# cloneofsimo/paint-with-words-sd

Measured on NVIDIA H100. Metric: unet_steps_per_sec_512sq_cfg, higher is better.
Workload: dtype f16

## Files before the change

paint_with_words_sd_b200/csrc/attn_tc.cuh:

```cuda
#pragma once
#include "mma_sm90.cuh"
#include "pww_common.cuh"
#include "xattn_core.cuh"

namespace pww {
namespace fa {

constexpr int kThreads = core::kThreads;
constexpr int kBM = core::kBM;
constexpr int kBN = 64;

template <int D>
struct Cfg {
  using T_ = core::Tile<D>;
  static constexpr uint32_t KVBYTES = kBN * T_::LD * 2;
  static constexpr uint32_t OFF_KV = T_::QBYTES;
  static constexpr uint32_t SMEM = T_::QBYTES + 2 * 2 * KVBYTES;
  static_assert(SMEM <= 232448, "shared memory budget");
};

template <typename E>
struct Params {
  const E* q;
  const E* k;
  const E* v;
  E* out;
  int B, H, N;
  int64_t bs, rs;
  int64_t o_bs, o_rs;
  float scale;
};

template <int D, typename E>
constexpr int kMinBlocks = (D == 80 && std::is_same_v<E, __nv_bfloat16>) ? 1 : 0;

template <int D, typename E>
__global__ void __launch_bounds__(kThreads, kMinBlocks<D, E>) attn_fwd_kernel(const Params<E> p) {
  using C = core::Tile<D>;
  using CF = Cfg<D>;
  extern __shared__ __align__(128) unsigned char smem[];
  const uint32_t smem0 = ptx::smem_u32(smem);
  const int warp = threadIdx.x >> 5, lane = threadIdx.x & 31;
  const int qtiles = (p.N + kBM - 1) / kBM;
  const int bh = blockIdx.x / qtiles, qt = blockIdx.x - bh * qtiles;
  const int b = bh / p.H, h = bh - b * p.H;
  const int row_base = qt * kBM;
  const E* qb = p.q + (int64_t)b * p.bs + h * D;
  const E* kb = p.k + (int64_t)b * p.bs + h * D;
  const E* vb = p.v + (int64_t)b * p.bs + h * D;
  const int ntiles = (p.N + kBN - 1) / kBN;
  auto issue_kv = [&](int j) {
    const uint32_t st = smem0 + CF::OFF_KV + (j & 1) * 2 * CF::KVBYTES;
    const int rows = p.N - j * kBN < kBN ? p.N - j * kBN : kBN;
    core::load_rows<D>(st, kb + (int64_t)j * kBN * p.rs, p.rs, kBN, rows);
    core::load_rows<D>(st + CF::KVBYTES, vb + (int64_t)j * kBN * p.rs, p.rs, kBN, rows);
    ptx::cp_async_commit();
  };
  {
    const int rows = p.N - row_base < kBM ? p.N - row_base : kBM;
    core::load_rows<D>(smem0, qb + (int64_t)row_base * p.rs, p.rs, kBM, rows);
  }
  issue_kv(0);
  uint32_t qa[C::KS][4];
  float o[C::NT][4], m0, m1, l0, l1;
  core::warp_online_begin<D>(o, m0, m1, l0, l1);
  const float sl2 = p.scale * 1.4426950408889634f;
  const uint32_t qs = smem0 + (uint32_t)(warp * 16 * C::LD) * 2u;
#pragma unroll 1
  for (int jt = 0; jt < ntiles; ++jt) {
    if (jt + 1 < ntiles) {
      issue_kv(jt + 1);
      ptx::cp_async_wait<1>();
    } else {
      ptx::cp_async_wait<0>();
    }
    __syncthreads();
    if (jt == 0) {
#pragma unroll
      for (int kk = 0; kk < C::KS; ++kk)
        ptx::ldsm_x4(qs + (uint32_t)((lane & 15) * C::LD + kk * 16 + (lane >> 4) * 8) * 2u, qa[kk][0], qa[kk][1], qa[kk][2], qa[kk][3]);
    }
    const uint32_t ks = smem0 + CF::OFF_KV + (jt & 1) * 2 * CF::KVBYTES, vs = ks + CF::KVBYTES;
    float s[kBN / 8][4];
#pragma unroll
    for (int j = 0; j < kBN / 8; ++j) s[j][0] = s[j][1] = s[j][2] = s[j][3] = 0.f;
#pragma unroll
    for (int kk = 0; kk < C::KS; ++kk) {
#pragma unroll
      for (int jp = 0; jp < kBN / 16; ++jp) {
        const int t = 16 * jp + (lane & 7) + ((lane >> 4) << 3), d = kk * 16 + ((lane >> 3) & 1) * 8;
        uint32_t b0, b1, b2, b3;
        ptx::ldsm_x4(ks + (uint32_t)(t * C::LD + d) * 2u, b0, b1, b2, b3);
        ptx::mma16816<E>(s[2 * jp], qa[kk], b0, b1);
        ptx::mma16816<E>(s[2 * jp + 1], qa[kk], b2, b3);
      }
    }
    core::warp_online_chunk<D, E>(s, p.N - jt * kBN, sl2, vs, lane, o, m0, m1, l0, l1);
    __syncthreads();
  }
  core::warp_online_end<D>(o, l0, l1);
  core::warp_store<D>(o, smem + warp * 16 * C::LD * 2, lane, p.out + (int64_t)b * p.o_bs + h * D, p.o_rs,
                      row_base + warp * 16, p.N);
}

template <int D, typename E>
cudaError_t launch(const void* q, const void* k, const void* v, void* out, int B, int H, int N, int64_t bs, int64_t rs,
                   int64_t o_bs, int64_t o_rs, float scale, cudaStream_t s) {
  using CF = Cfg<D>;
  Params<E> p;
  p.q = (const E*)q; p.k = (const E*)k; p.v = (const E*)v; p.out = (E*)out;
  p.B = B; p.H = H; p.N = N; p.bs = bs; p.rs = rs; p.o_bs = o_bs; p.o_rs = o_rs; p.scale = scale;
  const cudaError_t e = allow_dynamic_smem<attn_fwd_kernel<D, E>>(CF::SMEM);
  if (e != cudaSuccess) return e;
  const long long grid = (long long)B * H * ((N + kBM - 1) / kBM);
  if (grid > 0x7fffffffLL) return cudaErrorInvalidConfiguration;
  attn_fwd_kernel<D, E><<<(unsigned)grid, kThreads, CF::SMEM, s>>>(p);
  return cudaGetLastError();
}

}
}
```

paint_with_words_sd_b200/csrc/mma_sm90.cuh:

```cuda
#pragma once
#include <cuda_runtime.h>
#include <stdint.h>

#include <type_traits>

#include "pww_common.cuh"

namespace pww {
namespace ptx {

__device__ __forceinline__ uint32_t smem_u32(const void* p) { return (uint32_t)__cvta_generic_to_shared(p); }

__device__ __forceinline__ void cp_async16(uint32_t dst, const void* src, uint32_t src_bytes) {
  asm volatile("cp.async.cg.shared.global [%0], [%1], 16, %2;" ::"r"(dst), "l"(src), "r"(src_bytes) : "memory");
}
__device__ __forceinline__ void cp_async_commit() { asm volatile("cp.async.commit_group;" ::: "memory"); }
template <int N>
__device__ __forceinline__ void cp_async_wait() { asm volatile("cp.async.wait_group %0;" ::"n"(N) : "memory"); }

__device__ __forceinline__ void ldsm_x4(uint32_t addr, uint32_t& r0, uint32_t& r1, uint32_t& r2, uint32_t& r3) {
  asm volatile("ldmatrix.sync.aligned.m8n8.x4.shared.b16 {%0, %1, %2, %3}, [%4];"
               : "=r"(r0), "=r"(r1), "=r"(r2), "=r"(r3) : "r"(addr));
}
__device__ __forceinline__ void ldsm_x4_t(uint32_t addr, uint32_t& r0, uint32_t& r1, uint32_t& r2, uint32_t& r3) {
  asm volatile("ldmatrix.sync.aligned.m8n8.x4.trans.shared.b16 {%0, %1, %2, %3}, [%4];"
               : "=r"(r0), "=r"(r1), "=r"(r2), "=r"(r3) : "r"(addr));
}
__device__ __forceinline__ void ldsm_x2_t(uint32_t addr, uint32_t& r0, uint32_t& r1) {
  asm volatile("ldmatrix.sync.aligned.m8n8.x2.trans.shared.b16 {%0, %1}, [%2];" : "=r"(r0), "=r"(r1) : "r"(addr));
}

template <typename E>
__device__ __forceinline__ void mma16816(float* c, const uint32_t* a, uint32_t b0, uint32_t b1) {
  static_assert(std::is_same_v<E, __half> || std::is_same_v<E, __nv_bfloat16>, "fp16 or bf16 operands");
  if constexpr (std::is_same_v<E, __half>) {
    asm volatile(
        "mma.sync.aligned.m16n8k16.row.col.f32.f16.f16.f32 {%0, %1, %2, %3}, {%4, %5, %6, %7}, {%8, %9}, "
        "{%0, %1, %2, %3};"
        : "+f"(c[0]), "+f"(c[1]), "+f"(c[2]), "+f"(c[3])
        : "r"(a[0]), "r"(a[1]), "r"(a[2]), "r"(a[3]), "r"(b0), "r"(b1));
  } else {
    asm volatile(
        "mma.sync.aligned.m16n8k16.row.col.f32.bf16.bf16.f32 {%0, %1, %2, %3}, {%4, %5, %6, %7}, {%8, %9}, "
        "{%0, %1, %2, %3};"
        : "+f"(c[0]), "+f"(c[1]), "+f"(c[2]), "+f"(c[3])
        : "r"(a[0]), "r"(a[1]), "r"(a[2]), "r"(a[3]), "r"(b0), "r"(b1));
  }
}

__device__ __forceinline__ float ex2(float x) {
  float y;
  asm("ex2.approx.ftz.f32 %0, %1;" : "=f"(y) : "f"(x));
  return y;
}
template <typename E>
__device__ __forceinline__ uint32_t pack2(float lo, float hi) {
  const typename Elem<E>::E2 h = Elem<E>::from_float2(lo, hi);
  return *reinterpret_cast<const uint32_t*>(&h);
}
template <typename E>
__device__ __forceinline__ float2 unpack2(uint32_t v) {
  return Elem<E>::to_float2(*reinterpret_cast<const typename Elem<E>::E2*>(&v));
}
__device__ __forceinline__ unsigned long long ld_acquire_gpu_u64(const unsigned long long* p) {
  unsigned long long v;
  asm volatile("ld.acquire.gpu.global.u64 %0, [%1];" : "=l"(v) : "l"(p) : "memory");
  return v;
}

}
}
```

paint_with_words_sd_b200/csrc/xattn_core.cuh:

```cuda
#pragma once
#include "mma_sm90.cuh"
#include "pww_common.cuh"

namespace pww {
namespace core {

constexpr int kBM = 128;
constexpr int kTP = 80;
constexpr int kWarps = 8;
constexpr int kThreads = kWarps * 32;

template <int D>
struct Tile {
  static_assert(D == 40 || D == 64 || D == 80 || D == 160, "head dims of SD1.5 (40 / 80 / 160) and SD2.x (64)");
  static constexpr int DP = (D + 15) / 16 * 16;
  static constexpr int LD = DP + 8;
  static constexpr int KS = DP / 16;
  static constexpr int NT = D / 8;
  static constexpr uint32_t QBYTES = kBM * LD * 2;
  static constexpr uint32_t KBYTES = kTP * LD * 2;
};

template <int D, typename E>
__device__ __forceinline__ void load_rows(uint32_t dst, const E* src, int64_t rs, int nrows, int valid) {
  using C = Tile<D>;
  constexpr int CH = C::DP / 8, DCH = D / 8;
  for (int idx = threadIdx.x; idx < nrows * CH; idx += blockDim.x) {
    const int r = idx / CH, c = idx - r * CH;
    const bool ok = r < valid && c < DCH;
    ptx::cp_async16(dst + (uint32_t)(r * C::LD + c * 8) * 2u, ok ? (const void*)(src + (int64_t)r * rs + c * 8) : (const void*)src,
                    ok ? 16u : 0u);
  }
}

template <int D, typename E>
__device__ __forceinline__ void warp_qk(uint32_t qs, uint32_t ks, int lane, float (&s)[10][4]) {
  using C = Tile<D>;
#pragma unroll
  for (int j = 0; j < 10; ++j) s[j][0] = s[j][1] = s[j][2] = s[j][3] = 0.f;
#pragma unroll
  for (int kk = 0; kk < C::KS; ++kk) {
    uint32_t a[4];
    ptx::ldsm_x4(qs + (uint32_t)((lane & 15) * C::LD + kk * 16 + (lane >> 4) * 8) * 2u, a[0], a[1], a[2], a[3]);
#pragma unroll
    for (int jp = 0; jp < 5; ++jp) {
      const int t = 16 * jp + (lane & 7) + ((lane >> 4) << 3), d = kk * 16 + ((lane >> 3) & 1) * 8;
      uint32_t b0, b1, b2, b3;
      ptx::ldsm_x4(ks + (uint32_t)(t * C::LD + d) * 2u, b0, b1, b2, b3);
      ptx::mma16816<E>(s[2 * jp], a, b0, b1);
      ptx::mma16816<E>(s[2 * jp + 1], a, b2, b3);
    }
  }
}

__device__ __forceinline__ int tok(int j, int e, int lane) { return 8 * j + 2 * (lane & 3) + (e & 1); }

template <int D, typename E>
__device__ __forceinline__ void warp_store(const float (&o)[Tile<D>::NT][4], unsigned char* stage, int lane, E* out,
                                           int64_t o_rs, int row0, int N) {
  using C = Tile<D>;
  __syncwarp();
  const int g = lane >> 2, q = lane & 3;
#pragma unroll
  for (int j = 0; j < C::NT; ++j) {
    *reinterpret_cast<uint32_t*>(stage + (g * C::LD + 8 * j + 2 * q) * 2) = ptx::pack2<E>(o[j][0], o[j][1]);
    *reinterpret_cast<uint32_t*>(stage + ((g + 8) * C::LD + 8 * j + 2 * q) * 2) = ptx::pack2<E>(o[j][2], o[j][3]);
  }
  __syncwarp();
  for (int idx = lane; idx < 16 * C::NT; idx += 32) {
    const int r = idx / C::NT, c = idx - r * C::NT;
    if (row0 + r < N)
      *reinterpret_cast<uint4*>(out + (int64_t)(row0 + r) * o_rs + c * 8) =
          *reinterpret_cast<const uint4*>(stage + (r * C::LD + c * 8) * 2);
  }
  __syncwarp();
}

constexpr int kChunk = 77;
constexpr int kMaxChunks = 3;
__host__ __device__ __forceinline__ constexpr int chunks_of(int T) { return T <= kTP ? 1 : T / kChunk; }
__host__ __device__ __forceinline__ constexpr bool supported_keys(int T) {
  return T <= kTP || T == 2 * kChunk || T == kMaxChunks * kChunk;
}
template <int KC>
__host__ __device__ __forceinline__ constexpr int chunk_keys(int T) { return KC == 1 ? T : kChunk; }

template <int D, int KC, typename E>
__device__ __forceinline__ void load_operands(uint32_t st, const XattnParams<E>& p, int b, int h, int tile, bool with_v) {
  using C = Tile<D>;
  const int rows = p.N - tile * kBM;
  load_rows<D>(st, p.q + (int64_t)b * p.q_bs + (int64_t)tile * kBM * p.q_rs + h * D, p.q_rs, kBM, rows < kBM ? rows : kBM);
  const int kv = chunk_keys<KC>(p.T);
#pragma unroll 1
  for (int c = 0; c < KC; ++c) {
    const int64_t off = (int64_t)b * p.k_bs + (int64_t)c * kChunk * p.k_rs + h * D;
    load_rows<D>(st + C::QBYTES + c * C::KBYTES, p.k + off, p.k_rs, kTP, kv);
    if (with_v) load_rows<D>(st + C::QBYTES + (KC + c) * C::KBYTES, p.v + off, p.k_rs, kTP, kv);
  }
}

template <int D>
__device__ __forceinline__ void warp_online_begin(float (&o)[Tile<D>::NT][4], float& m0, float& m1, float& l0, float& l1) {
#pragma unroll
  for (int j = 0; j < Tile<D>::NT; ++j) o[j][0] = o[j][1] = o[j][2] = o[j][3] = 0.f;
  m0 = m1 = -INFINITY;
  l0 = l1 = 0.f;
}

struct NoPHook {
  template <int NK>
  __device__ __forceinline__ void operator()(const uint32_t (&)[NK][4], float, float) const {}
};

template <int D, typename E, int NJ, typename Hook = NoPHook>
__device__ __forceinline__ void warp_online_chunk(float (&s)[NJ][4], int kv, float sl2, uint32_t vs, int lane,
                                                  float (&o)[Tile<D>::NT][4], float& m0, float& m1, float& l0, float& l1,
                                                  const Hook& hook = Hook{}) {
  static_assert(NJ % 2 == 0, "P V takes two n-tiles of P per k-step");
  using C = Tile<D>;
  float t0 = -INFINITY, t1 = -INFINITY;
#pragma unroll
  for (int j = 0; j < NJ; ++j)
#pragma unroll
    for (int e = 0; e < 4; ++e) {
      if (tok(j, e, lane) >= kv) s[j][e] = -INFINITY;
      if (e < 2) t0 = fmaxf(t0, s[j][e]); else t1 = fmaxf(t1, s[j][e]);
    }
  t0 = fmaxf(t0, __shfl_xor_sync(0xffffffffu, t0, 1));
  t0 = fmaxf(t0, __shfl_xor_sync(0xffffffffu, t0, 2));
  t1 = fmaxf(t1, __shfl_xor_sync(0xffffffffu, t1, 1));
  t1 = fmaxf(t1, __shfl_xor_sync(0xffffffffu, t1, 2));
  const float mn0 = fmaxf(m0, t0), mn1 = fmaxf(m1, t1);
  const float a0 = ptx::ex2((m0 - mn0) * sl2), a1 = ptx::ex2((m1 - mn1) * sl2);
  m0 = mn0; m1 = mn1;
  const float n0 = -mn0 * sl2, n1 = -mn1 * sl2;
  uint32_t pa[NJ / 2][4];
  float r0 = 0.f, r1 = 0.f;
#pragma unroll
  for (int j = 0; j < NJ; ++j) {
    const uint32_t p01 = ptx::pack2<E>(ptx::ex2(fmaf(s[j][0], sl2, n0)), ptx::ex2(fmaf(s[j][1], sl2, n0)));
    const uint32_t p23 = ptx::pack2<E>(ptx::ex2(fmaf(s[j][2], sl2, n1)), ptx::ex2(fmaf(s[j][3], sl2, n1)));
    const float2 f01 = ptx::unpack2<E>(p01), f23 = ptx::unpack2<E>(p23);
    r0 += f01.x + f01.y;
    r1 += f23.x + f23.y;
    pa[j >> 1][(j & 1) * 2] = p01;
    pa[j >> 1][(j & 1) * 2 + 1] = p23;
  }
  l0 = l0 * a0 + r0;
  l1 = l1 * a1 + r1;
#pragma unroll
  for (int j = 0; j < C::NT; ++j) {
    o[j][0] *= a0; o[j][1] *= a0; o[j][2] *= a1; o[j][3] *= a1;
  }
#pragma unroll
  for (int kk = 0; kk < NJ / 2; ++kk) {
    const int t = 16 * kk + (lane & 7) + ((lane >> 3) & 1) * 8;
#pragma unroll
    for (int jp = 0; jp < C::NT / 2; ++jp) {
      uint32_t b0, b1, b2, b3;
      ptx::ldsm_x4_t(vs + (uint32_t)(t * C::LD + 16 * jp + (lane >> 4) * 8) * 2u, b0, b1, b2, b3);
      ptx::mma16816<E>(o[2 * jp], pa[kk], b0, b1);
      ptx::mma16816<E>(o[2 * jp + 1], pa[kk], b2, b3);
    }
    if constexpr (C::NT & 1) {
      uint32_t b0, b1;
      ptx::ldsm_x2_t(vs + (uint32_t)(t * C::LD + 8 * (C::NT - 1)) * 2u, b0, b1);
      ptx::mma16816<E>(o[C::NT - 1], pa[kk], b0, b1);
    }
  }
  hook(pa, a0, a1);
}

template <int D>
__device__ __forceinline__ void warp_online_end(float (&o)[Tile<D>::NT][4], float l0, float l1) {
  l0 += __shfl_xor_sync(0xffffffffu, l0, 1);
  l0 += __shfl_xor_sync(0xffffffffu, l0, 2);
  l1 += __shfl_xor_sync(0xffffffffu, l1, 1);
  l1 += __shfl_xor_sync(0xffffffffu, l1, 2);
  const float i0 = 1.f / l0, i1 = 1.f / l1;
#pragma unroll
  for (int j = 0; j < Tile<D>::NT; ++j) {
    o[j][0] *= i0; o[j][1] *= i0; o[j][2] *= i1; o[j][3] *= i1;
  }
}

constexpr int kRegions = 16;

template <typename E, int NK>
__device__ __forceinline__ void warp_region_chunk(const uint32_t (&pa)[NK][4], float a0, float a1, const int8_t* rt,
                                                  int lane, float (&rm)[2][4]) {
#pragma unroll
  for (int j = 0; j < 2; ++j) {
    rm[j][0] *= a0; rm[j][1] *= a0; rm[j][2] *= a1; rm[j][3] *= a1;
  }
  const int r = lane >> 2;
#pragma unroll
  for (int kk = 0; kk < NK; ++kk) {
    const int t = 16 * kk + 2 * (lane & 3);
    const int i0 = __ldg(rt + t), i1 = __ldg(rt + t + 1), i2 = __ldg(rt + t + 8), i3 = __ldg(rt + t + 9);
#pragma unroll
    for (int j = 0; j < 2; ++j) {
      const int slot = r + 8 * j;
      const uint32_t b0 = ptx::pack2<E>(i0 == slot ? 1.f : 0.f, i1 == slot ? 1.f : 0.f);
      const uint32_t b1 = ptx::pack2<E>(i2 == slot ? 1.f : 0.f, i3 == slot ? 1.f : 0.f);
      ptx::mma16816<E>(rm[j], pa[kk], b0, b1);
    }
  }
}

__device__ __forceinline__ void warp_region_add(const float (&rm)[2][4], float l0, float l1, float* acc, int row0, int N,
                                                int lane) {
  l0 += __shfl_xor_sync(0xffffffffu, l0, 1);
  l0 += __shfl_xor_sync(0xffffffffu, l0, 2);
  l1 += __shfl_xor_sync(0xffffffffu, l1, 1);
  l1 += __shfl_xor_sync(0xffffffffu, l1, 2);
  const float inv[2] = {1.f / l0, 1.f / l1};
  const int g = lane >> 2, q = lane & 3;
#pragma unroll
  for (int hf = 0; hf < 2; ++hf) {
    const int row = row0 + g + 8 * hf;
    if (row >= N) continue;
    float* a = acc + (int64_t)row * kRegions + 2 * q;
#pragma unroll
    for (int j = 0; j < 2; ++j) {
      a[8 * j] += rm[j][2 * hf] * inv[hf];
      a[8 * j + 1] += rm[j][2 * hf + 1] * inv[hf];
    }
  }
}

template <typename E>
__device__ __forceinline__ void warp_stat(const float (&s)[10][4], int T, int rows_left, int lane, bool is_max, float& vmax,
                                          float& sum, float& sumsq) {
  const int g = lane >> 2;
#pragma unroll
  for (int j = 0; j < 10; ++j)
#pragma unroll
    for (int e = 0; e < 4; ++e) {
      const bool ok = tok(j, e, lane) < T && (g + (e >> 1) * 8) < rows_left;
      if (is_max) {
        if (ok) vmax = fmaxf(vmax, s[j][e]);
      } else if (ok) {
        const float h = round_to<E>(s[j][e]);
        sum += h;
        sumsq = fmaf(h, h, sumsq);
      }
    }
}

__device__ __forceinline__ void warp_reduce_stat(double& m, double& a, double& q) {
#pragma unroll
  for (int o = 16; o > 0; o >>= 1) {
    m = fmax(m, __shfl_xor_sync(0xffffffffu, m, o));
    a += __shfl_xor_sync(0xffffffffu, a, o);
    q += __shfl_xor_sync(0xffffffffu, q, o);
  }
}

template <typename E>
__device__ __forceinline__ float stat_value(const XattnParams<E>& p, bool is_max, double m, double a, double q) {
  const double cnt = (double)p.H * (double)p.N * (double)p.T;
  double r;
  if (is_max) {
    r = m;
  } else {
    const double var = (q - a * a / cnt) / (cnt - 1.0);
    r = sqrt(var > 0.0 ? var : 0.0);
  }
  return round_to<E>((float)r);
}

}
}
```

Baseline: 160.0.

## Port self-attention kernel to Hopper wgmma with 3-stage KV ring

Replaces the mma.sync warp-level flash attention with warpgroup wgmma: Q and K/V are staged in 128B-swizzled shared memory, QK^T uses shared-shared wgmma, and PV uses register-A wgmma. It adds a 3-stage cp.async ring and overlaps the next tile's QK^T with the current tile's softmax and PV. Block size grows to 2 warpgroups covering 128 query rows. The aim is higher tensor-core throughput and better latency hiding, at the cost of more shared memory, higher register pressure, and complex fence ordering.

After: 160.7, median of 6. About the same (+0.5%).

```diff
diff --git a/paint_with_words_sd_b200/csrc/attn_tc.cuh b/paint_with_words_sd_b200/csrc/attn_tc.cuh
--- a/paint_with_words_sd_b200/csrc/attn_tc.cuh
+++ b/paint_with_words_sd_b200/csrc/attn_tc.cuh
@@ -6,17 +6,26 @@
 namespace pww {
 namespace fa {
 
-constexpr int kThreads = core::kThreads;
-constexpr int kBM = core::kBM;
+constexpr int kWarpgroups = 2;
+constexpr int kThreads = kWarpgroups * 128;
+constexpr int kBM = kWarpgroups * 64;
 constexpr int kBN = 64;
+constexpr int kStages = 3;
+constexpr uint32_t kAtom = 1024;
 
 template <int D>
 struct Cfg {
-  using T_ = core::Tile<D>;
-  static constexpr uint32_t KVBYTES = kBN * T_::LD * 2;
-  static constexpr uint32_t OFF_KV = T_::QBYTES;
-  static constexpr uint32_t SMEM = T_::QBYTES + 2 * 2 * KVBYTES;
+  static constexpr int DP = core::Tile<D>::DP;
+  static constexpr int KS = DP / 16;
+  static constexpr int CB = (DP + 63) / 64;
+  static constexpr uint32_t QBLK = kBM * 128;
+  static constexpr uint32_t KBLK = kBN * 128;
+  static constexpr uint32_t QBYTES = CB * QBLK;
+  static constexpr uint32_t KVBYTES = CB * KBLK;
+  static constexpr uint32_t STAGE = 2 * KVBYTES;
+  static constexpr uint32_t SMEM = kAtom + QBYTES + kStages * STAGE;
   static_assert(SMEM <= 232448, "shared memory budget");
+  static_assert(kBM * core::Tile<D>::LD * 2 <= QBYTES + kStages * STAGE, "epilogue staging");
 };
 
 template <typename E>
@@ -31,76 +40,153 @@
   float scale;
 };
 
+__device__ __forceinline__ uint32_t sw128_offset(int r, int c, uint32_t blk) {
+  return (uint32_t)(c >> 3) * blk + (uint32_t)r * 128u + ((uint32_t)((c & 7) ^ (r & 7)) << 4);
+}
+
+template <int D, int ROWS, int NT, typename E>
+__device__ __forceinline__ void load_tiles(uint32_t dst, uint32_t tstride, uint32_t blk, const E* const (&src)[NT],
+                                           int64_t rs, int valid) {
+  constexpr int CH = D / 8, PER = ROWS * CH, TOTAL = NT * PER;
+#pragma unroll 1
+  for (int it = 0; it < (TOTAL + kThreads - 1) / kThreads; ++it) {
+    const int idx = threadIdx.x + it * kThreads;
+    if (TOTAL % kThreads == 0 || idx < TOTAL) {
+      const int t = idx / PER, i = idx - t * PER;
+      const int r = i / CH, c = i - r * CH;
+      const E* s = src[0];
+#pragma unroll
+      for (int u = 1; u < NT; ++u) s = t == u ? src[u] : s;
+      const bool ok = r < valid;
+      ptx::cp_async16(dst + (uint32_t)t * tstride + sw128_offset(r, c, blk),
+                      ok ? (const void*)(s + (int64_t)r * rs + c * 8) : (const void*)s, ok ? 16u : 0u);
+    }
+  }
+}
+
+template <int D>
+__device__ __forceinline__ void zero_pad_columns(unsigned char* tile, int rows, uint32_t blk) {
+  constexpr int CH = D / 8, PCH = Cfg<D>::DP / 8 - CH;
+  if constexpr (PCH > 0) {
+    for (int idx = threadIdx.x; idx < rows * PCH; idx += kThreads) {
+      const int r = idx / PCH, c = CH + idx - r * PCH;
+      *reinterpret_cast<uint4*>(tile + sw128_offset(r, c, blk)) = make_uint4(0u, 0u, 0u, 0u);
+    }
+  }
+}
+
+template <int D>
+constexpr int kMinBlocks = D == 40 ? 2 : 1;
+
 template <int D, typename E>
-constexpr int kMinBlocks = (D == 80 && std::is_same_v<E, __nv_bfloat16>) ? 1 : 0;
-
-template <int D, typename E>
-__global__ void __launch_bounds__(kThreads, kMinBlocks<D, E>) attn_fwd_kernel(const Params<E> p) {
+__global__ void __launch_bounds__(kThreads, kMinBlocks<D>) attn_fwd_kernel(const Params<E> p) {
   using C = core::Tile<D>;
   using CF = Cfg<D>;
-  extern __shared__ __align__(128) unsigned char smem[];
+  extern __shared__ __align__(1024) unsigned char smem[];
   const uint32_t smem0 = ptx::smem_u32(smem);
-  const int warp = threadIdx.x >> 5, lane = threadIdx.x & 31;
+  const uint32_t base = (smem0 + kAtom - 1) & ~(kAtom - 1);
+  const uint32_t qs = base, ring = base + CF::QBYTES;
+  const int warp = threadIdx.x >> 5, lane = threadIdx.x & 31, wg = threadIdx.x >> 7;
   const int qtiles = (p.N + kBM - 1) / kBM;
   const int bh = blockIdx.x / qtiles, qt = blockIdx.x - bh * qtiles;
   const int b = bh / p.H, h = bh - b * p.H;
   const int row_base = qt * kBM;
-  const E* qb = p.q + (int64_t)b * p.bs + h * D;
   const E* kb = p.k + (int64_t)b * p.bs + h * D;
   const E* vb = p.v + (int64_t)b * p.bs + h * D;
   const int ntiles = (p.N + kBN - 1) / kBN;
+  auto stage = [&](int j) { return ring + (uint32_t)(j % kStages) * CF::STAGE; };
   auto issue_kv = [&](int j) {
-    const uint32_t st = smem0 + CF::OFF_KV + (j & 1) * 2 * CF::KVBYTES;
-    const int rows = p.N - j * kBN < kBN ? p.N - j * kBN : kBN;
-    core::load_rows<D>(st, kb + (int64_t)j * kBN * p.rs, p.rs, kBN, rows);
-    core::load_rows<D>(st + CF::KVBYTES, vb + (int64_t)j * kBN * p.rs, p.rs, kBN, rows);
+    if (j < ntiles) {
+      const int rows = p.N - j * kBN < kBN ? p.N - j * kBN : kBN;
+      const E* const src[2] = {kb + (int64_t)j * kBN * p.rs, vb + (int64_t)j * kBN * p.rs};
+      load_tiles<D, kBN, 2>(stage(j), CF::KVBYTES, CF::KBLK, src, p.rs, rows);
+    }
     ptx::cp_async_commit();
   };
+  auto issue_qk = [&](float (&s)[kBN / 8][4], int j) {
+    const uint32_t qw = qs + (uint32_t)wg * 64u * 128u, ks = stage(j);
+    ptx::wgmma_fence();
+#pragma unroll
+    for (int kk = 0; kk < CF::KS; ++kk) {
+      const uint32_t col = (uint32_t)(kk & 3) * 32u;
+      const uint64_t da = ptx::smem_desc_sw128(qw + (uint32_t)(kk >> 2) * CF::QBLK + col, 16u, kAtom);
+      const uint64_t db = ptx::smem_desc_sw128(ks + (uint32_t)(kk >> 2) * CF::KBLK + col, 16u, kAtom);
+      ptx::Wgmma<kBN>::template ss<E>(&s[0][0], da, db, kk > 0);
+    }
+    ptx::wgmma_commit();
+  };
+  auto issue_pv = [&](float (&o)[C::NT][4], const uint32_t (&pa)[kBN / 16][4], int j) {
+    const uint32_t vs = stage(j) + CF::KVBYTES;
+    ptx::wgmma_fence();
+#pragma unroll
+    for (int kk = 0; kk < kBN / 16; ++kk) {
+      const uint32_t row = (uint32_t)kk * 16u * 128u;
+#pragma unroll
+      for (int cb = 0; cb < CF::CB; ++cb) {
+        constexpr int kLast = D - 64 * (CF::CB - 1);
+        const uint64_t dv = ptx::smem_desc_sw128(vs + (uint32_t)cb * CF::KBLK + row, kAtom, kAtom);
+        if (cb + 1 < CF::CB)
+          ptx::Wgmma<64>::template rs_tb<E>(&o[8 * cb][0], pa[kk], dv);
+        else
+          ptx::Wgmma<kLast>::template rs_tb<E>(&o[8 * cb][0], pa[kk], dv);
+      }
+    }
+    ptx::wgmma_commit();
+  };
+
   {
+    unsigned char* const tiles = smem + (base - smem0);
+    zero_pad_columns<D>(tiles, kBM, CF::QBLK);
+#pragma unroll 1
+    for (int st = 0; st < kStages; ++st) zero_pad_columns<D>(tiles + CF::QBYTES + st * CF::STAGE, kBN, CF::KBLK);
     const int rows = p.N - row_base < kBM ? p.N - row_base : kBM;
-    core::load_rows<D>(smem0, qb + (int64_t)row_base * p.rs, p.rs, kBM, rows);
+    const E* const src[1] = {p.q + (int64_t)b * p.bs + (int64_t)row_base * p.rs + h * D};
+    load_tiles<D, kBM, 1>(qs, 0u, CF::QBLK, src, p.rs, rows);
   }
   issue_kv(0);
-  uint32_t qa[C::KS][4];
+  issue_kv(1);
+  ptx::cp_async_wait<1>();
+  ptx::fence_proxy_async();
+  __syncthreads();
+  float s[kBN / 8][4];
+  issue_qk(s, 0);
+  ptx::wgmma_wait<0>();
+  ptx::fence_operands(s);
+  issue_kv(2);
+  ptx::cp_async_wait<1>();
+  ptx::fence_proxy_async();
+  __syncthreads();
+
   float o[C::NT][4], m0, m1, l0, l1;
   core::warp_online_begin<D>(o, m0, m1, l0, l1);
   const float sl2 = p.scale * 1.4426950408889634f;
-  const uint32_t qs = smem0 + (uint32_t)(warp * 16 * C::LD) * 2u;
 #pragma unroll 1
   for (int jt = 0; jt < ntiles; ++jt) {
-    if (jt + 1 < ntiles) {
-      issue_kv(jt + 1);
-      ptx::cp_async_wait<1>();
-    } else {
-      ptx::cp_async_wait<0>();
-    }
+    float sn[kBN / 8][4];
+    const bool next = jt + 1 < ntiles;
+    if (next) issue_qk(sn, jt + 1);
+    uint32_t pa[kBN / 16][4];
+    float a0, a1;
+    core::warp_online_p<D, E, kBN / 8>(s, p.N - jt * kBN, sl2, lane, o, m0, m1, l0, l1, pa, a0, a1);
+    issue_pv(o, pa, jt);
+    ptx::wgmma_wait<0>();
+    ptx::fence_operands(o);
+    ptx::fence_operands(pa);
+    if (next) {
+      ptx::fence_operands(sn);
+#pragma unroll
+      for (int j = 0; j < kBN / 8; ++j)
+#pragma unroll
+        for (int e = 0; e < 4; ++e) s[j][e] = sn[j][e];
+    }
+    ptx::cp_async_wait<0>();
+    ptx::fence_proxy_async();
     __syncthreads();
-    if (jt == 0) {
-#pragma unroll
-      for (int kk = 0; kk < C::KS; ++kk)
-        ptx::ldsm_x4(qs + (uint32_t)((lane & 15) * C::LD + kk * 16 + (lane >> 4) * 8) * 2u, qa[kk][0], qa[kk][1], qa[kk][2], qa[kk][3]);
-    }
-    const uint32_t ks = smem0 + CF::OFF_KV + (jt & 1) * 2 * CF::KVBYTES, vs = ks + CF::KVBYTES;
-    float s[kBN / 8][4];
-#pragma unroll
-    for (int j = 0; j < kBN / 8; ++j) s[j][0] = s[j][1] = s[j][2] = s[j][3] = 0.f;
-#pragma unroll
-    for (int kk = 0; kk < C::KS; ++kk) {
-#pragma unroll
-      for (int jp = 0; jp < kBN / 16; ++jp) {
-        const int t = 16 * jp + (lane & 7) + ((lane >> 4) << 3), d = kk * 16 + ((lane >> 3) & 1) * 8;
-        uint32_t b0, b1, b2, b3;
-        ptx::ldsm_x4(ks + (uint32_t)(t * C::LD + d) * 2u, b0, b1, b2, b3);
-        ptx::mma16816<E>(s[2 * jp], qa[kk], b0, b1);
-        ptx::mma16816<E>(s[2 * jp + 1], qa[kk], b2, b3);
-      }
-    }
-    core::warp_online_chunk<D, E>(s, p.N - jt * kBN, sl2, vs, lane, o, m0, m1, l0, l1);
-    __syncthreads();
+    issue_kv(jt + 3);
   }
   core::warp_online_end<D>(o, l0, l1);
-  core::warp_store<D>(o, smem + warp * 16 * C::LD * 2, lane, p.out + (int64_t)b * p.o_bs + h * D, p.o_rs,
-                      row_base + warp * 16, p.N);
+  core::warp_store<D>(o, smem + (base - smem0) + warp * 16 * C::LD * 2, lane, p.out + (int64_t)b * p.o_bs + h * D,
+                      p.o_rs, row_base + warp * 16, p.N);
 }
 
 template <int D, typename E>
diff --git a/paint_with_words_sd_b200/csrc/mma_sm90.cuh b/paint_with_words_sd_b200/csrc/mma_sm90.cuh
--- a/paint_with_words_sd_b200/csrc/mma_sm90.cuh
+++ b/paint_with_words_sd_b200/csrc/mma_sm90.cuh
@@ -48,6 +48,129 @@
   }
 }
 
+__device__ __forceinline__ void fence_proxy_async() { asm volatile("fence.proxy.async.shared::cta;" ::: "memory"); }
+__device__ __forceinline__ void wgmma_fence() { asm volatile("wgmma.fence.sync.aligned;" ::: "memory"); }
+__device__ __forceinline__ void wgmma_commit() { asm volatile("wgmma.commit_group.sync.aligned;" ::: "memory"); }
+template <int N>
+__device__ __forceinline__ void wgmma_wait() { asm volatile("wgmma.wait_group.sync.aligned %0;" ::"n"(N) : "memory"); }
+template <int R, int C>
+__device__ __forceinline__ void fence_operands(float (&r)[R][C]) {
+#pragma unroll
+  for (int i = 0; i < R; ++i)
+#pragma unroll
+    for (int j = 0; j < C; ++j) asm volatile("" : "+f"(r[i][j])::"memory");
+}
+template <int R, int C>
+__device__ __forceinline__ void fence_operands(uint32_t (&r)[R][C]) {
+#pragma unroll
+  for (int i = 0; i < R; ++i)
+#pragma unroll
+    for (int j = 0; j < C; ++j) asm volatile("" : "+r"(r[i][j])::"memory");
+}
+
+__host__ __device__ constexpr uint64_t smem_desc_sw128(uint32_t addr, uint32_t lbo, uint32_t sbo) {
+  return (uint64_t)((addr & 0x3FFFFu) >> 4) | (uint64_t)((lbo & 0x3FFFFu) >> 4) << 16 |
+         (uint64_t)((sbo & 0x3FFFFu) >> 4) << 32 | 1ull << 62;
+}
+
+template <int N>
+struct Wgmma;
+template <>
+struct Wgmma<16> {
+  template <typename E>
+  static __device__ __forceinline__ void rs_tb(float* d, const uint32_t* a, uint64_t b) {
+    if constexpr (std::is_same_v<E, __half>)
+      asm volatile("{\n.reg .pred p;\nsetp.ne.b32 p, %13, 0;\n"
+                   "wgmma.mma_async.sync.aligned.m64n16k16.f32.f16.f16 {%0, %1, %2, %3, %4, %5, %6, %7}, {%8, %9, %10, %11}, %12, p, 1, 1, 1;\n}\n"
+                   : "+f"(d[0]), "+f"(d[1]), "+f"(d[2]), "+f"(d[3]), "+f"(d[4]), "+f"(d[5]), "+f"(d[6]), "+f"(d[7])
+                   : "r"(a[0]), "r"(a[1]), "r"(a[2]), "r"(a[3]), "l"(b), "r"(1));
+    else
+      asm volatile("{\n.reg .pred p;\nsetp.ne.b32 p, %13, 0;\n"
+                   "wgmma.mma_async.sync.aligned.m64n16k16.f32.bf16.bf16 {%0, %1, %2, %3, %4, %5, %6, %7}, {%8, %9, %10, %11}, %12, p, 1, 1, 1;\n}\n"
+                   : "+f"(d[0]), "+f"(d[1]), "+f"(d[2]), "+f"(d[3]), "+f"(d[4]), "+f"(d[5]), "+f"(d[6]), "+f"(d[7])
+                   : "r"(a[0]), "r"(a[1]), "r"(a[2]), "r"(a[3]), "l"(b), "r"(1));
+  }
+};
+template <>
+struct Wgmma<32> {
+  template <typename E>
+  static __device__ __forceinline__ void rs_tb(float* d, const uint32_t* a, uint64_t b) {
+    if constexpr (std::is_same_v<E, __half>)
+      asm volatile("{\n.reg .pred p;\nsetp.ne.b32 p, %21, 0;\n"
+                   "wgmma.mma_async.sync.aligned.m64n32k16.f32.f16.f16 {%0, %1, %2, %3, %4, %5, %6, %7, %8, %9, %10, %11, %12, %13, %14, %15}, {%16, %17, %18, %19}, %20, p, 1, 1, 1;\n}\n"
+                   : "+f"(d[0]), "+f"(d[1]), "+f"(d[2]), "+f"(d[3]), "+f"(d[4]), "+f"(d[5]), "+f"(d[6]), "+f"(d[7]),
+                   "+f"(d[8]), "+f"(d[9]), "+f"(d[10]), "+f"(d[11]), "+f"(d[12]), "+f"(d[13]), "+f"(d[14]), "+f"(d[15])
+                   : "r"(a[0]), "r"(a[1]), "r"(a[2]), "r"(a[3]), "l"(b), "r"(1));
+    else
+      asm volatile("{\n.reg .pred p;\nsetp.ne.b32 p, %21, 0;\n"
+                   "wgmma.mma_async.sync.aligned.m64n32k16.f32.bf16.bf16 {%0, %1, %2, %3, %4, %5, %6, %7, %8, %9, %10, %11, %12, %13, %14, %15}, {%16, %17, %18, %19}, %20, p, 1, 1, 1;\n}\n"
+                   : "+f"(d[0]), "+f"(d[1]), "+f"(d[2]), "+f"(d[3]), "+f"(d[4]), "+f"(d[5]), "+f"(d[6]), "+f"(d[7]),
+                   "+f"(d[8]), "+f"(d[9]), "+f"(d[10]), "+f"(d[11]), "+f"(d[12]), "+f"(d[13]), "+f"(d[14]), "+f"(d[15])
+                   : "r"(a[0]), "r"(a[1]), "r"(a[2]), "r"(a[3]), "l"(b), "r"(1));
+  }
+};
+template <>
+struct Wgmma<40> {
+  template <typename E>
+  static __device__ __forceinline__ void rs_tb(float* d, const uint32_t* a, uint64_t b) {
+    if constexpr (std::is_same_v<E, __half>)
+      asm volatile("{\n.reg .pred p;\nsetp.ne.b32 p, %25, 0;\n"
+                   "wgmma.mma_async.sync.aligned.m64n40k16.f32.f16.f16 {%0, %1, %2, %3, %4, %5, %6, %7, %8, %9, %10, %11, %12, %13, %14, %15, %16, %17, %18, %19}, {%20, %21, %22, %23}, %24, p, 1, 1, 1;\n}\n"
+                   : "+f"(d[0]), "+f"(d[1]), "+f"(d[2]), "+f"(d[3]), "+f"(d[4]), "+f"(d[5]), "+f"(d[6]), "+f"(d[7]),
+                   "+f"(d[8]), "+f"(d[9]), "+f"(d[10]), "+f"(d[11]), "+f"(d[12]), "+f"(d[13]), "+f"(d[14]), "+f"(d[15]),
+                   "+f"(d[16]), "+f"(d[17]), "+f"(d[18]), "+f"(d[19])
+                   : "r"(a[0]), "r"(a[1]), "r"(a[2]), "r"(a[3]), "l"(b), "r"(1));
+    else
+      asm volatile("{\n.reg .pred p;\nsetp.ne.b32 p, %25, 0;\n"
+                   "wgmma.mma_async.sync.aligned.m64n40k16.f32.bf16.bf16 {%0, %1, %2, %3, %4, %5, %6, %7, %8, %9, %10, %11, %12, %13, %14, %15, %16, %17, %18, %19}, {%20, %21, %22, %23}, %24, p, 1, 1, 1;\n}\n"
+                   : "+f"(d[0]), "+f"(d[1]), "+f"(d[2]), "+f"(d[3]), "+f"(d[4]), "+f"(d[5]), "+f"(d[6]), "+f"(d[7]),
+                   "+f"(d[8]), "+f"(d[9]), "+f"(d[10]), "+f"(d[11]), "+f"(d[12]), "+f"(d[13]), "+f"(d[14]), "+f"(d[15]),
+                   "+f"(d[16]), "+f"(d[17]), "+f"(d[18]), "+f"(d[19])
+                   : "r"(a[0]), "r"(a[1]), "r"(a[2]), "r"(a[3]), "l"(b), "r"(1));
+  }
+};
+template <>
+struct Wgmma<64> {
+  template <typename E>
+  static __device__ __forceinline__ void ss(float* d, uint64_t a, uint64_t b, int acc) {
+    if constexpr (std::is_same_v<E, __half>)
+      asm volatile("{\n.reg .pred p;\nsetp.ne.b32 p, %34, 0;\n"
+                   "wgmma.mma_async.sync.aligned.m64n64k16.f32.f16.f16 {%0, %1, %2, %3, %4, %5, %6, %7, %8, %9, %10, %11, %12, %13, %14, %15, %16, %17, %18, %19, %20, %21, %22, %23, %24, %25, %26, %27, %28, %29, %30, %31}, %32, %33, p, 1, 1, 0, 0;\n}\n"
+                   : "+f"(d[0]), "+f"(d[1]), "+f"(d[2]), "+f"(d[3]), "+f"(d[4]), "+f"(d[5]), "+f"(d[6]), "+f"(d[7]),
+                   "+f"(d[8]), "+f"(d[9]), "+f"(d[10]), "+f"(d[11]), "+f"(d[12]), "+f"(d[13]), "+f"(d[14]), "+f"(d[15]),
+                   "+f"(d[16]), "+f"(d[17]), "+f"(d[18]), "+f"(d[19]), "+f"(d[20]), "+f"(d[21]), "+f"(d[22]), "+f"(d[23]),
+                   "+f"(d[24]), "+f"(d[25]), "+f"(d[26]), "+f"(d[27]), "+f"(d[28]), "+f"(d[29]), "+f"(d[30]), "+f"(d[31])
+                   : "l"(a), "l"(b), "r"(acc));
+    else
+      asm volatile("{\n.reg .pred p;\nsetp.ne.b32 p, %34, 0;\n"
+                   "wgmma.mma_async.sync.aligned.m64n64k16.f32.bf16.bf16 {%0, %1, %2, %3, %4, %5, %6, %7, %8, %9, %10, %11, %12, %13, %14, %15, %16, %17, %18, %19, %20, %21, %22, %23, %24, %25, %26, %27, %28, %29, %30, %31}, %32, %33, p, 1, 1, 0, 0;\n}\n"
+                   : "+f"(d[0]), "+f"(d[1]), "+f"(d[2]), "+f"(d[3]), "+f"(d[4]), "+f"(d[5]), "+f"(d[6]), "+f"(d[7]),
+                   "+f"(d[8]), "+f"(d[9]), "+f"(d[10]), "+f"(d[11]), "+f"(d[12]), "+f"(d[13]), "+f"(d[14]), "+f"(d[15]),
+                   "+f"(d[16]), "+f"(d[17]), "+f"(d[18]), "+f"(d[19]), "+f"(d[20]), "+f"(d[21]), "+f"(d[22]), "+f"(d[23]),
+                   "+f"(d[24]), "+f"(d[25]), "+f"(d[26]), "+f"(d[27]), "+f"(d[28]), "+f"(d[29]), "+f"(d[30]), "+f"(d[31])
+                   : "l"(a), "l"(b), "r"(acc));
+  }
+  template <typename E>
+  static __device__ __forceinline__ void rs_tb(float* d, const uint32_t* a, uint64_t b) {
+    if constexpr (std::is_same_v<E, __half>)
+      asm volatile("{\n.reg .pred p;\nsetp.ne.b32 p, %37, 0;\n"
+                   "wgmma.mma_async.sync.aligned.m64n64k16.f32.f16.f16 {%0, %1, %2, %3, %4, %5, %6, %7, %8, %9, %10, %11, %12, %13, %14, %15, %16, %17, %18, %19, %20, %21, %22, %23, %24, %25, %26, %27, %28, %29, %30, %31}, {%32, %33, %34, %35}, %36, p, 1, 1, 1;\n}\n"
+                   : "+f"(d[0]), "+f"(d[1]), "+f"(d[2]), "+f"(d[3]), "+f"(d[4]), "+f"(d[5]), "+f"(d[6]), "+f"(d[7]),
+                   "+f"(d[8]), "+f"(d[9]), "+f"(d[10]), "+f"(d[11]), "+f"(d[12]), "+f"(d[13]), "+f"(d[14]), "+f"(d[15]),
+                   "+f"(d[16]), "+f"(d[17]), "+f"(d[18]), "+f"(d[19]), "+f"(d[20]), "+f"(d[21]), "+f"(d[22]), "+f"(d[23]),
+                   "+f"(d[24]), "+f"(d[25]), "+f"(d[26]), "+f"(d[27]), "+f"(d[28]), "+f"(d[29]), "+f"(d[30]), "+f"(d[31])
+                   : "r"(a[0]), "r"(a[1]), "r"(a[2]), "r"(a[3]), "l"(b), "r"(1));
+    else
+      asm volatile("{\n.reg .pred p;\nsetp.ne.b32 p, %37, 0;\n"
+                   "wgmma.mma_async.sync.aligned.m64n64k16.f32.bf16.bf16 {%0, %1, %2, %3, %4, %5, %6, %7, %8, %9, %10, %11, %12, %13, %14, %15, %16, %17, %18, %19, %20, %21, %22, %23, %24, %25, %26, %27, %28, %29, %30, %31}, {%32, %33, %34, %35}, %36, p, 1, 1, 1;\n}\n"
+                   : "+f"(d[0]), "+f"(d[1]), "+f"(d[2]), "+f"(d[3]), "+f"(d[4]), "+f"(d[5]), "+f"(d[6]), "+f"(d[7]),
+                   "+f"(d[8]), "+f"(d[9]), "+f"(d[10]), "+f"(d[11]), "+f"(d[12]), "+f"(d[13]), "+f"(d[14]), "+f"(d[15]),
+                   "+f"(d[16]), "+f"(d[17]), "+f"(d[18]), "+f"(d[19]), "+f"(d[20]), "+f"(d[21]), "+f"(d[22]), "+f"(d[23]),
+                   "+f"(d[24]), "+f"(d[25]), "+f"(d[26]), "+f"(d[27]), "+f"(d[28]), "+f"(d[29]), "+f"(d[30]), "+f"(d[31])
+                   : "r"(a[0]), "r"(a[1]), "r"(a[2]), "r"(a[3]), "l"(b), "r"(1));
+  }
+};
+
 __device__ __forceinline__ float ex2(float x) {
   float y;
   asm("ex2.approx.ftz.f32 %0, %1;" : "=f"(y) : "f"(x));
diff --git a/paint_with_words_sd_b200/csrc/xattn_core.cuh b/paint_with_words_sd_b200/csrc/xattn_core.cuh
--- a/paint_with_words_sd_b200/csrc/xattn_core.cuh
+++ b/paint_with_words_sd_b200/csrc/xattn_core.cuh
@@ -112,18 +112,24 @@
   __device__ __forceinline__ void operator()(const uint32_t (&)[NK][4], float, float) const {}
 };
 
-template <int D, typename E, int NJ, typename Hook = NoPHook>
-__device__ __forceinline__ void warp_online_chunk(float (&s)[NJ][4], int kv, float sl2, uint32_t vs, int lane,
-                                                  float (&o)[Tile<D>::NT][4], float& m0, float& m1, float& l0, float& l1,
-                                                  const Hook& hook = Hook{}) {
+template <int D, typename E, int NJ>
+__device__ __forceinline__ void warp_online_p(float (&s)[NJ][4], int kv, float sl2, int lane, float (&o)[Tile<D>::NT][4],
+                                              float& m0, float& m1, float& l0, float& l1, uint32_t (&pa)[NJ / 2][4],
+                                              float& a0, float& a1) {
   static_assert(NJ % 2 == 0, "P V takes two n-tiles of P per k-step");
   using C = Tile<D>;
+  if (kv < NJ * 8) {
+#pragma unroll
+    for (int j = 0; j < NJ; ++j)
+#pragma unroll
+      for (int e = 0; e < 4; ++e)
+        if (tok(j, e, lane) >= kv) s[j][e] = -INFINITY;
+  }
   float t0 = -INFINITY, t1 = -INFINITY;
 #pragma unroll
   for (int j = 0; j < NJ; ++j)
 #pragma unroll
     for (int e = 0; e < 4; ++e) {
-      if (tok(j, e, lane) >= kv) s[j][e] = -INFINITY;
       if (e < 2) t0 = fmaxf(t0, s[j][e]); else t1 = fmaxf(t1, s[j][e]);
     }
   t0 = fmaxf(t0, __shfl_xor_sync(0xffffffffu, t0, 1));
@@ -131,10 +137,10 @@
   t1 = fmaxf(t1, __shfl_xor_sync(0xffffffffu, t1, 1));
   t1 = fmaxf(t1, __shfl_xor_sync(0xffffffffu, t1, 2));
   const float mn0 = fmaxf(m0, t0), mn1 = fmaxf(m1, t1);
-  const float a0 = ptx::ex2((m0 - mn0) * sl2), a1 = ptx::ex2((m1 - mn1) * sl2);
+  a0 = ptx::ex2((m0 - mn0) * sl2);
+  a1 = ptx::ex2((m1 - mn1) * sl2);
   m0 = mn0; m1 = mn1;
   const float n0 = -mn0 * sl2, n1 = -mn1 * sl2;
-  uint32_t pa[NJ / 2][4];
   float r0 = 0.f, r1 = 0.f;
 #pragma unroll
   for (int j = 0; j < NJ; ++j) {
@@ -152,6 +158,16 @@
   for (int j = 0; j < C::NT; ++j) {
     o[j][0] *= a0; o[j][1] *= a0; o[j][2] *= a1; o[j][3] *= a1;
   }
+}
+
+template <int D, typename E, int NJ, typename Hook = NoPHook>
+__device__ __forceinline__ void warp_online_chunk(float (&s)[NJ][4], int kv, float sl2, uint32_t vs, int lane,
+                                                  float (&o)[Tile<D>::NT][4], float& m0, float& m1, float& l0, float& l1,
+                                                  const Hook& hook = Hook{}) {
+  using C = Tile<D>;
+  uint32_t pa[NJ / 2][4];
+  float a0, a1;
+  warp_online_p<D, E, NJ>(s, kv, sl2, lane, o, m0, m1, l0, l1, pa, a0, a1);
 #pragma unroll
   for (int kk = 0; kk < NJ / 2; ++kk) {
     const int t = 16 * kk + (lane & 7) + ((lane >> 3) & 1) * 8;
```
